# barlettacarmen/CrCNN

Hardware: AMD Instinct MI355X
Metric: encrypted images/sec (higher is better)
Workload: dtype u64

## Files before the change

crcnn_amd/csrc/kernels_mfma.hip:

```cpp
#include "kernels.h"
#include "limbred.h"
#include <cstdlib>

typedef int v4i __attribute__((ext_vector_type(4)));
typedef int v16i __attribute__((ext_vector_type(16)));
typedef signed char i8;

#define NPL 7
#define TILE_B (NPL * 64 * 32)

struct MfmaArgs {
    const i8 *xl; const i8 *wl; u64 *ys; const ModParams *mods; const u64 *bias;
    int xcdmap;
    int mfast;
    i8 *xl_out; int lp2; unsigned zdp_out;
    int n, k, B, zdp, npos, yd, xs, ys_, yf, yo, P, F, Fp, zblks, ksteps, M, mtiles, ntiles;
    unsigned img_bytes; unsigned long long wslot_bytes; int ksteps_real;
    int flat, S, zdc; unsigned fplane;
    int acc0[8][13];
    u64 qinv[8];
};

__device__ __forceinline__ void limb_digits(u64 r, u64 q, int (&d)[NPL])
{
    long long v = r > (q >> 1) ? (long long)r - (long long)q : (long long)r;
#pragma unroll
    for (int l = 0; l < NPL; l++) { d[l] = (int)(signed char)(v & 0xff); v = (v - d[l]) >> 8; }
}

template <int NST>
__global__ void __launch_bounds__(256) __attribute__((amdgpu_waves_per_eu(1, 1))) mfma_mac_kernel(MfmaArgs a)
{
    extern __shared__ __attribute__((aligned(16))) i8 lds[];
    const int lane = threadIdx.x & 63, wave = __builtin_amdgcn_readfirstlane(threadIdx.x >> 6), wm = wave >> 1, wn = wave & 1;
    const int slots = a.n * a.k, per = a.mtiles * a.ntiles;
    int g = blockIdx.x, slot, tile;
    if ((slots & 7) == 0) { const int xcd = g & 7, r = g >> 3; slot = xcd * (slots >> 3) + r / per; tile = r % per; }
    else { slot = g / per; tile = g % per; }
    const int mt = a.mfast ? tile % a.mtiles : tile / a.ntiles, nt = a.mfast ? tile / a.mtiles : tile % a.ntiles;
    const int i = slot / a.n, s = slot % a.n;
    const int m0 = mt * 64, f0 = nt * 64;
    const ModParams m = a.mods[i];
    const u64 qinv = a.qinv[i];
    const i8 *xs = a.xl + (size_t)slot * a.B * a.img_bytes;
    const i8 *ws = a.wl + (size_t)slot * a.wslot_bytes + (size_t)f0 * 32;
    u32 src_off[7];
#pragma unroll
    for (int j = 0; j < 7; j++) {
        const int pc = wave + 4 * j;
        if (pc < 14) {
            const int c16 = pc * 64 + lane;
            const int plane = c16 >> 7, row = (c16 >> 1) & 63, half = c16 & 1;
            const int mm = min(m0 + row, a.M - 1);
            const int b = mm / (2 * a.P), p = (mm >> 1) % a.P, c = mm & 1;
            const int ox = p / a.yo, oy = p % a.yo;
            src_off[j] = a.npos == 1 ? (u32)(plane * a.zblks * (2 * a.B) + mm) * 32 + half * 16
                       : a.flat ? (u32)b * a.img_bytes + (u32)(plane * a.fplane + (c * a.npos + (ox * a.xs) * a.yd + oy * a.ys_) * a.zdc + half * 16)
                                : (u32)b * a.img_bytes + (u32)(plane * (a.npos * 2 * a.zdp) + (((ox * a.xs) * a.yd + oy * a.ys_) * 2 + c) * a.zdp + half * 16);
        } else src_off[j] = (u32)(((pc - 14) >> 1) * (a.Fp * 32) + ((pc - 14) & 1) * 1024 + lane * 16);
    }
    const int kreal = a.ksteps_real;
    auto issue = [&](int ks) {
        const int ka = min(ks, kreal - 1);
        const int tap = ka / a.zblks, zb = ka - tap * a.zblks;
        const int kx = tap / a.yf, ky = tap - kx * a.yf;
        const int fkx = ka / a.S;
        const u32 delta = a.npos == 1 ? (u32)zb * (2 * a.B) * 32 : a.flat ? (u32)(fkx * a.yd * a.zdc + (ka - fkx * a.S) * 32) : (u32)((kx * a.yd + ky) * 2 * a.zdp + zb * 32);
        i8 *dst = lds + (ks % NST) * (2 * TILE_B);
        const i8 *wt = ws + (size_t)ks * (NPL * a.Fp * 32);
#pragma unroll
        for (int j = 0; j < 7; j++) {
            const int pc = wave + 4 * j;
            const i8 *src = pc < 14 ? xs + src_off[j] + delta : wt + src_off[j];
            __builtin_amdgcn_global_load_lds((const __attribute__((address_space(1))) void *)src, (__attribute__((address_space(3))) void *)(dst + pc * 1024), 16, 0, 0);
        }
    };
    v4i acc[2][2][13];
#pragma unroll
    for (int rs = 0; rs < 2; rs++)
#pragma unroll
        for (int cs = 0; cs < 2; cs++)
#pragma unroll
            for (int d = 0; d < 13; d++) { const int b0 = a.acc0[i][d]; acc[rs][cs][d] = v4i{b0, b0, b0, b0}; }
    const int K = a.ksteps;
#pragma unroll
    for (int j = 0; j < NST - 2; j++) if (j < K) issue(j);
    const int kg = lane >> 4, r16 = lane & 15;
    const int fragA = (wm * 32 + r16) * 32 + (kg & 1) * 16, fragW = (wn * 32 + r16) * 32 + (kg & 1) * 16;
    for (int ks = 0; ks < K; ks += 2) {
        const int younger = min(NST - 4, K - 2 - ks);
        if (younger >= 1) __builtin_amdgcn_s_waitcnt(7 | (7 << 4) | (15 << 8));
        else __builtin_amdgcn_s_waitcnt(0 | (7 << 4) | (15 << 8));
        __syncthreads();
        __builtin_amdgcn_sched_barrier(0);
        if (ks + NST - 2 < K) { issue(ks + NST - 2); __builtin_amdgcn_sched_barrier(0); if (ks + NST - 1 < K) issue(ks + NST - 1); }
        __builtin_amdgcn_sched_barrier(0);
        const i8 *tA = lds + ((ks + (kg >> 1)) % NST) * (2 * TILE_B), *tW = tA + TILE_B;
        v4i w[2][NPL], av[2 * NPL];
        auto read_a = [&](int gi) { return *reinterpret_cast<const v4i *>(tA + (gi % NPL) * (64 * 32) + fragA + (gi / NPL) * (16 * 32)); };
#pragma unroll
        for (int cs = 0; cs < 2; cs++)
#pragma unroll
            for (int l = 0; l < NPL; l++) w[cs][l] = *reinterpret_cast<const v4i *>(tW + l * (64 * 32) + fragW + cs * (16 * 32));
        av[0] = read_a(0); av[1] = read_a(1);
        __builtin_amdgcn_sched_barrier(0);
#pragma unroll
        for (int gi = 0; gi < 2 * NPL; gi++) {
            const int rs = gi / NPL, l = gi % NPL;
#pragma unroll
            for (int cs = 0; cs < 2; cs++)
#pragma unroll
                for (int mm = 0; mm < NPL; mm++)
                    acc[rs][cs][l + mm] = __builtin_amdgcn_mfma_i32_16x16x64_i8(av[gi], w[cs][mm], acc[rs][cs][l + mm], 0, 0, 0);
            if (gi + 2 < 2 * NPL) av[gi + 2] = read_a(gi + 2);
            __builtin_amdgcn_sched_barrier(0);
        }
    }
    u64 *yslot = a.ys + (size_t)slot * a.B * a.F * (2 * a.P);
    const u32 P2 = 2 * a.P;
    const u32 RL = 64 * a.P;
    if (a.xl_out) __syncthreads();
#pragma unroll
    for (int rs = 0; rs < 2; rs++) {
        const u32 mbase = m0 + wm * 32 + rs * 16 + 4 * kg, bb = mbase / P2, rem = mbase - bb * P2;
#pragma unroll
        for (int cs = 0; cs < 2; cs++) {
            const int fl = wn * 32 + cs * 16 + r16, f = f0 + fl;
            const u64 bv = (a.bias && f < a.F) ? a.bias[((size_t)f * a.k + i) * a.n + s] : 0;
#pragma unroll
            for (int reg = 0; reg < 4; reg++) {
                int D[13];
#pragma unroll
                for (int d = 0; d < 13; d++) D[d] = acc[rs][cs][d][reg];
                u64 v = diag_reduce_w(D, m, qinv);
                if ((reg & 1) == 0) v = addmod(v, bv, m.q);
                if (a.xl_out) {
                    const u32 rt = wm * 32 + rs * 16 + 4 * kg + reg, bl = rt >> a.lp2, qq = rt & (P2 - 1);
                    const u64 dg = f < a.F ? balanced_digit_bytes(v, m.q) : 0;
                    i8 *sp = lds + (size_t)bl * (NPL * 2 * RL) + (qq & 1) * RL + fl * a.P + (qq >> 1);
#pragma unroll
                    for (int l = 0; l < NPL; l++) sp[(size_t)l * (2 * RL)] = (i8)(dg >> (8 * l));
                } else {
                    const u32 r = rem + reg, b = bb + (r >= P2) + (r >= 2 * P2);
                    if (mbase + reg < (u32)a.M && f < a.F) yslot[b * (u32)(a.F - 1) * P2 + (u32)f * P2 + mbase + reg] = v;
                }
                __builtin_amdgcn_sched_barrier(0);
            }
        }
    }
    if (a.xl_out) {
        __syncthreads();
        const u32 imgs = 64 >> a.lp2, b0 = (u32)m0 >> a.lp2, per_run = RL / 16, pieces = imgs * NPL * 2 * per_run;
        const u32 ch0 = (u32)f0 * a.P;
        for (u32 o = threadIdx.x; o < pieces; o += 256) {
            const u32 run = o / per_run, off = (o - run * per_run) * 16, bl = run / (NPL * 2), lc = run - bl * (NPL * 2);
            const u32 ch = ch0 + off;
            if (b0 + bl < (u32)a.B && ch < a.zdp_out)
                *reinterpret_cast<uint4 *>(a.xl_out + (size_t)slot * ((size_t)NPL * 2 * a.B * a.zdp_out)
                                           + ((size_t)((lc >> 1) * (a.zdp_out / 32) + (ch >> 5)) * (2 * a.B) + (b0 + bl) * 2 + (lc & 1)) * 32 + (ch & 31)) =
                    *reinterpret_cast<const uint4 *>(lds + (size_t)run * RL + off);
        }
    }
}

#define TILE_A (NPL * 64 * 32)
template <int NST, int MODE>
__global__ void __launch_bounds__(256) __attribute__((amdgpu_waves_per_eu(2, 2))) mfma_mac2w_kernel(MfmaArgs a)
{
    extern __shared__ __attribute__((aligned(16))) i8 lds[];
    const int lane = threadIdx.x & 63, wave = __builtin_amdgcn_readfirstlane(threadIdx.x >> 6), wm = wave >> 1, wn = wave & 1;
    const int slots = a.n * a.k;
    const int fast = a.xcdmap ? (int)(blockIdx.x >> 3) : (int)blockIdx.x, slow = (int)blockIdx.y;
    const int slot = a.xcdmap ? (int)(blockIdx.x & 7) * (slots >> 3) + (int)blockIdx.z : (int)blockIdx.z;
    const int mt = a.mfast ? fast : slow, nt = a.mfast ? slow : fast;
    const int lgn = __builtin_ctz(a.n), i = slot >> lgn, s = slot & (a.n - 1);
    const int m0 = mt * 64, f0 = nt * 32;
    if (f0 >= a.F) return;
    const ModParams m = a.mods[i];
    const u64 qinv = a.qinv[i];
    const i8 *xs = a.xl + (size_t)slot * a.B * a.img_bytes;
    const int kg = lane >> 4, r16 = lane & 15;
    const i8 *wlane = a.wl + (size_t)slot * a.wslot_bytes + (size_t)(f0 + wn * 16 + r16) * 32 + (kg & 1) * 16 + (size_t)(kg >> 1) * (NPL * a.Fp * 32);
    const int wplane = a.Fp * 32, wstep = NPL * a.Fp * 32;
    u32 src_off[4]; int pcs[4];
    {
        const int row = ((wave & 1) << 5) + (lane >> 1), half = lane & 1;
        const int mm = min(m0 + row, a.M - 1);
        const int b = mm / (2 * a.P), rem = mm - b * (2 * a.P), p = rem >> 1, c = rem & 1;
        const int ox = p / a.yo, oy = p - ox * a.yo;
        const u32 rowpart = MODE == 0 ? (u32)mm * 32 + half * 16
                          : MODE == 1 ? (u32)b * a.img_bytes + (u32)((c * a.npos + (ox * a.xs) * a.yd + oy * a.ys_) * a.zdc + half * 16)
                                   : (u32)b * a.img_bytes + (u32)((((ox * a.xs) * a.yd + oy * a.ys_) * 2 + c) * a.zdp + half * 16);
        const u32 pstride = MODE == 0 ? (u32)(a.zblks * (2 * a.B)) * 32 : MODE == 1 ? a.fplane : (u32)(a.npos * 2 * a.zdp);
#pragma unroll
        for (int j = 0; j < 4; j++) {
            pcs[j] = wave + 4 * j < 14 ? wave + 4 * j : wave + 8;
            src_off[j] = rowpart + (u32)(pcs[j] >> 1) * pstride;
        }
    }
    const int kreal = a.ksteps_real;
    int iss = 0, ibuf = 0, zb = 0, ky = 0, kx = 0;
    u32 delta = 0;
    auto issue_a = [&](int ks) {
        (void)ks;
        i8 *dst = lds + ibuf * TILE_A;
#pragma unroll
        for (int j = 0; j < 4; j++)
            __builtin_amdgcn_global_load_lds((const __attribute__((address_space(1))) void *)(xs + src_off[j] + delta), (__attribute__((address_space(3))) void *)(dst + pcs[j] * 1024), 16, 0, 0);
        iss++; ibuf = ibuf + 1 == NST ? 0 : ibuf + 1;
        if (iss < kreal) {
            if (MODE == 0) delta += (u32)(2 * a.B) * 32;
            else if (MODE == 1) { if (++zb == a.S) { zb = 0; kx++; } delta = (u32)(kx * a.yd * a.zdc + zb * 32); }
            else { if (++zb == a.zblks) { zb = 0; if (++ky == a.yf) { ky = 0; kx++; } } delta = (u32)((kx * a.yd + ky) * 2 * a.zdp + zb * 32); }
        }
    };
    auto load_w = [&](int ks, v4i (&w)[NPL]) {
        const i8 *pw = wlane + (size_t)ks * wstep;
#pragma unroll
        for (int l = 0; l < NPL; l++) w[l] = *reinterpret_cast<const v4i *>(pw + (size_t)l * wplane);
    };
    v4i acc[2][13];
#pragma unroll
    for (int rs = 0; rs < 2; rs++)
#pragma unroll
        for (int d = 0; d < 13; d++) { const int b0 = a.acc0[i][d]; acc[rs][d] = v4i{b0, b0, b0, b0}; }
    const int K = a.ksteps;
    const int fragA = (wm * 32 + r16) * 32 + (kg & 1) * 16;
    auto dstep = [&](int ks, v4i (&wuse)[NPL], v4i (&wload)[NPL]) {
        if (ks + 2 < K) __builtin_amdgcn_s_waitcnt(11 | (7 << 4) | (15 << 8));
        else __builtin_amdgcn_s_waitcnt(0 | (7 << 4) | (15 << 8));
        __syncthreads();
        __builtin_amdgcn_sched_barrier(0);
        if (ks + 3 < K) issue_a(ks + 3);
        __builtin_amdgcn_sched_barrier(0);
        if (ks + 4 < K) { load_w(ks + 4, wload); __builtin_amdgcn_sched_barrier(0); issue_a(ks + 4); }
        __builtin_amdgcn_sched_barrier(0);
        const i8 *tA = lds + ((ks + (kg >> 1)) % NST) * TILE_A;
        v4i av[2 * NPL];
        auto read_a = [&](int gi) { return *reinterpret_cast<const v4i *>(tA + (gi % NPL) * (64 * 32) + fragA + (gi / NPL) * (16 * 32)); };
        av[0] = read_a(0); av[1] = read_a(1); av[2] = read_a(2);
        __builtin_amdgcn_sched_barrier(0);
#pragma unroll
        for (int gi = 0; gi < 2 * NPL; gi++) {
            const int rs = gi / NPL, l = gi % NPL;
#pragma unroll
            for (int mm = 0; mm < NPL; mm++)
                acc[rs][l + mm] = __builtin_amdgcn_mfma_i32_16x16x64_i8(av[gi], wuse[mm], acc[rs][l + mm], 0, 0, 0);
            if (gi + 3 < 2 * NPL) av[gi + 3] = read_a(gi + 3);
            __builtin_amdgcn_sched_barrier(0);
        }
    };
    v4i w0[NPL], w1[NPL], w2[NPL];
    issue_a(0); if (1 < K) issue_a(1);
    __builtin_amdgcn_sched_barrier(0);
    load_w(0, w0);
    __builtin_amdgcn_sched_barrier(0);
    if (2 < K) { issue_a(2); __builtin_amdgcn_sched_barrier(0); load_w(2, w1); }
    __builtin_amdgcn_sched_barrier(0);
    for (int ks = 0; ks < K; ks += 6) {
        dstep(ks, w0, w2);
        if (ks + 2 < K) dstep(ks + 2, w1, w0);
        if (ks + 4 < K) dstep(ks + 4, w2, w1);
    }
    u64 *yslot = a.ys + (size_t)slot * a.B * a.F * (2 * a.P);
    const u32 P2 = 2 * a.P;
    const u32 RL = 32 * a.P;
    if (a.xl_out) __syncthreads();
    const int fl = wn * 16 + r16, f = f0 + fl;
    const u64 bv = (a.bias && f < a.F) ? a.bias[((size_t)f * a.k + i) * a.n + s] : 0;
    const u32 img_jump = (u32)(a.F - 1) * P2;
#pragma unroll
    for (int rs = 0; rs < 2; rs++) {
        const u32 mbase = m0 + wm * 32 + rs * 16 + 4 * kg, bb = mbase / P2, rem = mbase - bb * P2;
        const u32 idx0 = bb * img_jump + (u32)f * P2 + mbase;
#pragma unroll
        for (int reg = 0; reg < 4; reg++) {
            int D[13];
#pragma unroll
            for (int d = 0; d < 13; d++) D[d] = acc[rs][d][reg];
            u64 v = diag_reduce_w(D, m, qinv);
            if ((reg & 1) == 0) v = addmod(v, bv, m.q);
            if (a.xl_out) {
                const u32 rt = wm * 32 + rs * 16 + 4 * kg + reg, bl = rt >> a.lp2, qq = rt & (P2 - 1);
                const u64 dg = f < a.F ? balanced_digit_bytes(v, m.q) : 0;
                i8 *sp = lds + (size_t)bl * (NPL * 2 * RL) + (qq & 1) * RL + fl * a.P + (qq >> 1);
#pragma unroll
                for (int l = 0; l < NPL; l++) sp[(size_t)l * (2 * RL)] = (i8)(dg >> (8 * l));
            } else {
                const u32 r = rem + reg, jump = (r >= P2 ? img_jump : 0u) + (r >= 2 * P2 ? img_jump : 0u);
                if (mbase + reg < (u32)a.M && f < a.F) yslot[idx0 + reg + jump] = v;
            }
            __builtin_amdgcn_sched_barrier(0);
        }
    }
    if (a.xl_out) {
        __syncthreads();
        const u32 imgs = 64 >> a.lp2, b0 = (u32)m0 >> a.lp2, per_run = RL / 16, pieces = imgs * NPL * 2 * per_run;
        const u32 ch0 = (u32)f0 * a.P;
        for (u32 o = threadIdx.x; o < pieces; o += 256) {
            const u32 run = o / per_run, off = (o - run * per_run) * 16, bl = run / (NPL * 2), lc = run - bl * (NPL * 2);
            const u32 ch = ch0 + off;
            if (b0 + bl < (u32)a.B && ch < a.zdp_out)
                *reinterpret_cast<uint4 *>(a.xl_out + (size_t)slot * ((size_t)NPL * 2 * a.B * a.zdp_out)
                                           + ((size_t)((lc >> 1) * (a.zdp_out / 32) + (ch >> 5)) * (2 * a.B) + (b0 + bl) * 2 + (lc & 1)) * 32 + (ch & 31)) =
                    *reinterpret_cast<const uint4 *>(lds + (size_t)run * RL + off);
        }
    }
}

__global__ void __launch_bounds__(64) limb_pack_tensor_kernel(const u64 *x, i8 *xl, const ModParams *mods, int n, int k, int B, int zd, int zdp, int npos, int packed, int group,
                                                              int Btot, int b0, int flat_zdc, unsigned flat_img)
{
    const int sblocks = n / 64;
    const int sb = blockIdx.x % (sblocks * k), i = sb / sblocks, s = (sb % sblocks) * 64 + threadIdx.x;
    const int zblks = zdp / 32;
    const size_t items = (size_t)B * npos * 2 * zblks;
    const u64 q = mods[i].q;
    for (size_t r0 = (size_t)(blockIdx.x / (sblocks * k)) * group, u = 0; u < (size_t)group && r0 + u < items; u++) {
        size_t r = r0 + u;
        int zb, c, pos, b;
        if (npos == 1) { const size_t rows = (size_t)B * 2; zb = (int)(r / rows); r %= rows; c = (int)(r & 1); b = (int)(r >> 1); pos = 0; }
        else { zb = (int)(r % zblks); r /= zblks; c = (int)(r % 2); r /= 2; pos = (int)(r % npos); b = (int)(r / npos); }
        u32 pl[NPL][8];
#pragma unroll
        for (int l = 0; l < NPL; l++)
#pragma unroll
            for (int wv = 0; wv < 8; wv++) pl[l][wv] = 0;
#pragma unroll
        for (int z = 0; z < 32; z++) {
            const int zz = zb * 32 + z;
            if (zz < zd) {
                u64 v = x[((((size_t)b * zd * npos + (size_t)zz * npos + pos) * 2 + c) * k + i) * (size_t)n + s];
                if (packed) v = (v & 0xffffffffULL) | ((v >> 32) << 28);
                int d[NPL]; limb_digits(v, q, d);
#pragma unroll
                for (int l = 0; l < NPL; l++) pl[l][z >> 2] |= (u32)(d[l] & 0xff) << (8 * (z & 3));
            }
        }
        if (flat_zdc) {
            i8 *dstf = xl + (((size_t)i * n + s) * Btot + b0 + b) * (size_t)flat_img + ((size_t)c * npos + pos) * flat_zdc;
#pragma unroll
            for (int l = 0; l < NPL; l++) {
                u32 *o = reinterpret_cast<u32 *>(dstf + (size_t)l * 2 * npos * flat_zdc);
#pragma unroll
                for (int wv = 0; wv < 8; wv++) if (wv * 4 < flat_zdc) o[wv] = pl[l][wv];
            }
            continue;
        }
        i8 *dst = npos == 1 ? xl + ((size_t)i * n + s) * ((size_t)NPL * 2 * Btot * zdp) + ((size_t)zb * (2 * Btot) + (b0 + b) * 2 + c) * 32
                            : xl + (((size_t)i * n + s) * Btot + b0 + b) * ((size_t)NPL * npos * 2 * zdp) + ((size_t)pos * 2 + c) * zdp + zb * 32;
        const size_t plane_stride = npos == 1 ? (size_t)zblks * (2 * Btot) * 32 : (size_t)npos * 2 * zdp;
#pragma unroll
        for (int l = 0; l < NPL; l++) {
            uint4 *o = reinterpret_cast<uint4 *>(dst + (size_t)l * plane_stride);
            o[0] = make_uint4(pl[l][0], pl[l][1], pl[l][2], pl[l][3]); o[1] = make_uint4(pl[l][4], pl[l][5], pl[l][6], pl[l][7]);
        }
    }
}
#define TRG 4
#define TSL 32
__global__ void __launch_bounds__(256) limb_pack_dense_kernel(const u64 *x, i8 *xl, const ModParams *mods, int n, int k, int B, int zd, int zdp, int packed, int Btot, int b0)
{
    __shared__ __attribute__((aligned(16))) i8 st[TSL * NPL * TRG * 32];
    const int sblocks = n / TSL, zblks = zdp / 32, rgs = (2 * B + TRG - 1) / TRG;
    const int sb = blockIdx.x % (sblocks * k), i = sb / sblocks, s0 = (sb % sblocks) * TSL;
    size_t r = blockIdx.x / (sblocks * k);
    const int rg = (int)(r % rgs), zb = (int)(r / rgs);
    const u64 q = mods[i].q;
    const int lane = threadIdx.x & (TSL - 1), qrow = (threadIdx.x >> 5) & (TRG - 1), h = threadIdx.x >> 7, row = rg * TRG + qrow;
    {
        u32 pl[NPL][4];
#pragma unroll
        for (int l = 0; l < NPL; l++)
#pragma unroll
            for (int wv = 0; wv < 4; wv++) pl[l][wv] = 0;
        if (row < 2 * B) {
            const int b = row >> 1, c = row & 1, z0 = zb * 32 + h * 16;
            const u64 *src = x + ((((size_t)b * zd + z0) * 2 + c) * k + i) * (size_t)n + s0 + lane;
#pragma unroll
            for (int z = 0; z < 16; z++)
                if (z0 + z < zd) {
                    u64 v = src[(size_t)z * 2 * k * n];
                    if (packed) v = (v & 0xffffffffULL) | ((v >> 32) << 28);
                    int d[NPL]; limb_digits(v, q, d);
#pragma unroll
                    for (int l = 0; l < NPL; l++) pl[l][z >> 2] |= (u32)(d[l] & 0xff) << (8 * (z & 3));
                }
        }
        i8 *sp = st + (size_t)lane * (NPL * TRG * 32) + qrow * 32 + h * 16;
#pragma unroll
        for (int l = 0; l < NPL; l++) *reinterpret_cast<uint4 *>(sp + l * (TRG * 32)) = make_uint4(pl[l][0], pl[l][1], pl[l][2], pl[l][3]);
    }
    __syncthreads();
    const int pieces_per_run = TRG * 2, rows_here = min(TRG, 2 * B - rg * TRG);
    const size_t plane_stride = (size_t)zblks * (2 * Btot) * 32, slot_stride = (size_t)NPL * plane_stride;
    for (int o = threadIdx.x; o < TSL * NPL * pieces_per_run; o += 256) {
        const int run = o / pieces_per_run, part = o - run * pieces_per_run, sl = run / NPL, l = run - sl * NPL;
        if ((part >> 1) >= rows_here) continue;
        i8 *dst = xl + ((size_t)i * n + s0 + sl) * slot_stride + (size_t)l * plane_stride + ((size_t)zb * (2 * Btot) + (size_t)b0 * 2 + rg * TRG) * 32 + part * 16;
        *reinterpret_cast<uint4 *>(dst) = *reinterpret_cast<const uint4 *>(st + (size_t)run * (TRG * 32) + part * 16);
    }
}
#define WFG 4
#define WSL 32
__global__ void __launch_bounds__(256) limb_pack_weights_kernel(const u64 *w, i8 *wl, const ModParams *mods, int n, int k, int F, int Fz, int Fp, int zd, int zblks, int xf, int yf, int f0,
                                                                int flat_zdc, int S)
{
    __shared__ __attribute__((aligned(16))) i8 st[WSL * NPL * WFG * 32];
    const int sblocks = n / WSL, taps = xf * yf, steps = flat_zdc ? xf * S : taps * zblks;
    const int sb = blockIdx.x % (sblocks * k), i = sb / sblocks, s0 = (sb % sblocks) * WSL;
    size_t r = blockIdx.x / (sblocks * k);
    const int step = (int)(r % steps); const int fg = (int)(r / steps);
    const ModParams m = mods[i];
    const u64 R = barrett128(0, 1, m);
    const int lane = threadIdx.x & (WSL - 1), fq = (threadIdx.x >> 5) & (WFG - 1), h = threadIdx.x >> 7, f = fg * WFG + fq;
    {
        u32 pl[NPL][4];
#pragma unroll
        for (int l = 0; l < NPL; l++)
#pragma unroll
            for (int wv = 0; wv < 4; wv++) pl[l][wv] = 0;
        if (f < F) {
            int tap, ch, ky = 0, kx = 0;
            if (flat_zdc) { kx = step / S; const int j0 = (step - kx * S) * 32 + h * 16; ky = j0 / flat_zdc; ch = j0 - ky * flat_zdc; tap = kx * yf + ky; }
            else { tap = step / zblks; ch = (step - tap * zblks) * 32 + h * 16; }
#pragma unroll
            for (int z = 0; z < 16; z++) {
                if (ch < zd && (!flat_zdc || ky < yf)) {
                    const u64 v = mulmod(w[((((size_t)f * zd + ch) * taps + tap) * k + i) * (size_t)n + s0 + lane], R, m);
                    int d[NPL]; limb_digits(v, m.q, d);
#pragma unroll
                    for (int l = 0; l < NPL; l++) pl[l][z >> 2] |= (u32)(d[l] & 0xff) << (8 * (z & 3));
                }
                ch++;
                if (flat_zdc && ch == flat_zdc) { ch = 0; ky++; tap++; }
            }
        }
        i8 *sp = st + (size_t)lane * (NPL * WFG * 32) + fq * 32 + h * 16;
#pragma unroll
        for (int l = 0; l < NPL; l++) *reinterpret_cast<uint4 *>(sp + l * (WFG * 32)) = make_uint4(pl[l][0], pl[l][1], pl[l][2], pl[l][3]);
    }
    __syncthreads();
    const int pieces_per_run = WFG * 2, filters_here = min(WFG, Fz - fg * WFG);
    const size_t slot_stride = (size_t)((steps + 1) & ~1) * NPL * Fp * 32;
    for (int o = threadIdx.x; o < WSL * NPL * pieces_per_run; o += 256) {
        const int run = o / pieces_per_run, part = o - run * pieces_per_run, sl = run / NPL, l = run - sl * NPL;
        if ((part >> 1) >= filters_here) continue;
        i8 *dst = wl + ((size_t)i * n + s0 + sl) * slot_stride + (size_t)step * (NPL * Fp * 32) + (size_t)l * Fp * 32 + (size_t)(f0 + fg * WFG) * 32 + part * 16;
// ... 12 lines not shown
        const int sl = r * 4 + ty;
        const size_t e = e0 + tx;
        tile[sl][tx] = e < rows ? ys[((size_t)i * n + s0 + sl) * rows + e] : 0;
    }
    __syncthreads();
#pragma unroll
    for (int r = 0; r < 16; r++) {
        const int el = r * 4 + ty;
        const size_t e = e0 + el;
        if (e < rows) { u64 v = tile[tx][el]; if (pack_out) v = (v & 0x0fffffffULL) | ((v >> 28) << 32); y[(e * k + i) * (size_t)n + s0 + tx] = v; }
    }
}
__global__ void __launch_bounds__(256) slotmajor_to_limb_kernel(const u64 *ys, i8 *xl, const ModParams *mods, int n, int B, int zd, int zdp, size_t total)
{
    const size_t t = (size_t)blockIdx.x * blockDim.x + threadIdx.x;
    if (t >= total) return;
    const int zgs = zdp / 16;
    const int zg = (int)(t % zgs); size_t r = t / zgs; const int c = (int)(r % 2); r /= 2; const int b = (int)(r % B); const size_t slot = r / B;
    const u64 q = mods[slot / n].q;
    u32 pl[NPL][4];
#pragma unroll
    for (int l = 0; l < NPL; l++)
#pragma unroll
        for (int wv = 0; wv < 4; wv++) pl[l][wv] = 0;
    const u64 *src = ys + (slot * B + b) * (size_t)zd * 2 + c;
#pragma unroll
    for (int z = 0; z < 16; z++) {
        const int zz = zg * 16 + z;
        if (zz < zd) {
            int d[NPL]; limb_digits(src[(size_t)zz * 2], q, d);
#pragma unroll
            for (int l = 0; l < NPL; l++) pl[l][z >> 2] |= (u32)(d[l] & 0xff) << (8 * (z & 3));
        }
    }
    i8 *dst = xl + slot * ((size_t)NPL * 2 * B * zdp) + ((size_t)(zg >> 1) * (2 * B) + b * 2 + c) * 32 + (zg & 1) * 16;
#pragma unroll
    for (int l = 0; l < NPL; l++) *reinterpret_cast<uint4 *>(dst + (size_t)l * (zdp / 32) * (2 * B) * 32) = make_uint4(pl[l][0], pl[l][1], pl[l][2], pl[l][3]);
}

static inline int round_up(int v, int m) { return (v + m - 1) / m * m; }
int k_limb_flat_zdc(int zd);
static void limb_tables(const crc_ctx *c, int T, int (*acc0)[13], u64 *qinv)
{
    for (int i = 0; i < c->k; i++) { limb_bias_table(c->tabs[i].m.q, T, acc0[i]); qinv[i] = inverse_mod_2_64(c->tabs[i].m.q); }
}

bool k_limb_supported(const crc_ctx *c, int T)
{
    if (c->n < 64 || T > 18000) return false;
    for (int i = 0; i < c->k; i++) if (c->tabs[i].m.bits > 55) return false;
    return true;
}
int k_limb_flat_zdc(int zd) { return zd < 32 ? round_up(zd, 4) : 0; }
int k_limb_steps(int zd, int xf, int yf) { const int zdc = k_limb_flat_zdc(zd); return zdc ? xf * ((yf * zdc + 31) / 32) : xf * yf * (round_up(zd, 32) / 32); }
static size_t limb_img_bytes(int zd, int npos) { const int zdc = k_limb_flat_zdc(zd); return zdc ? (size_t)round_up(NPL * 2 * npos * zdc, 16) : (size_t)NPL * npos * 2 * round_up(zd, 32); }
size_t k_limb_tensor_bytes(const crc_ctx *c, int B, int zd, int npos)
{
    if (npos == 1) return (size_t)c->n * c->k * B * NPL * 2 * round_up(zd, 32);
    return (size_t)c->n * c->k * B * limb_img_bytes(zd, npos) + 64;
}
size_t k_limb_weights_bytes(const crc_ctx *c, int nf, int zd, int xf, int yf) { return (size_t)c->n * c->k * round_up(k_limb_steps(zd, xf, yf), 2) * NPL * round_up(nf, 64) * 32; }
size_t k_limb_result_words(const crc_ctx *c, int B, int nf, int P) { return (size_t)c->n * c->k * B * nf * P * 2; }

int k_limb_pack_tensor(crc_ctx *c, const u64 *x, i8 *xl, int B, int zd, int npos, bool packed, hipStream_t st, int Btot, int b0)
{
    if (Btot <= 0) { Btot = B; b0 = 0; }
    if (b0 < 0 || b0 + B > Btot) return CRC_ERR_INVALID_ARGUMENT;
    const int zdp = round_up(zd, 32);
    const int group = c->tune.limb_pack_group > 1 ? c->tune.limb_pack_group : (npos == 1 && (B * 2) % 4 == 0 ? 4 : 1);
    const size_t items = (size_t)B * npos * 2 * (zdp / 32);
    if (npos == 1 && c->tune.limb_pack_group <= 1) {
        const size_t blocks = (size_t)(c->n / TSL) * c->k * (zdp / 32) * ((2 * (size_t)B + TRG - 1) / TRG);
        if (blocks == 0) return CRC_OK;
        if (blocks > 0x7fffffffULL) return CRC_ERR_INVALID_ARGUMENT;
        hipLaunchKernelGGL(limb_pack_dense_kernel, dim3((unsigned)blocks), dim3(256), 0, st, x, xl, c->d_mods, c->n, c->k, B, zd, zdp, packed ? 1 : 0, Btot, b0);
        HIPCHK(hipGetLastError());
        return CRC_OK;
    }
    const size_t blocks = (size_t)(c->n / 64) * c->k * ((items + group - 1) / group);
    if (blocks == 0) return CRC_OK;
    if (blocks > 0x7fffffffULL) return CRC_ERR_INVALID_ARGUMENT;
    const int fz = npos > 1 ? k_limb_flat_zdc(zd) : 0;
    hipLaunchKernelGGL(limb_pack_tensor_kernel, dim3((unsigned)blocks), dim3(64), 0, st, x, xl, c->d_mods, c->n, c->k, B, zd, zdp, npos, packed ? 1 : 0, group, Btot, b0, fz,
                       (unsigned)limb_img_bytes(zd, npos));
    HIPCHK(hipGetLastError());
    return CRC_OK;
}
int k_limb_pack_weights(crc_ctx *c, const u64 *w, i8 *wl, int nf, int zd, int xf, int yf, hipStream_t st, int f0, int ft)
{
    if (ft < 0) ft = nf;
    if (f0 < 0 || ft < 1 || f0 + ft > nf) return CRC_ERR_INVALID_ARGUMENT;
    const int zblks = round_up(zd, 32) / 32, Fp = round_up(nf, 64), zdc = k_limb_flat_zdc(zd), S = zdc ? (yf * zdc + 31) / 32 : 0;
    const size_t step = (size_t)NPL * Fp * 32, steps = (size_t)k_limb_steps(zd, xf, yf), slot = (size_t)round_up((int)steps, 2) * step;
    if (f0 == 0 && (steps & 1)) HIPCHK(hipMemset2DAsync(wl + steps * step, slot, 0, step, (size_t)c->n * c->k, st));
    const int fz = f0 + ft == nf ? Fp - f0 : ft;
    const size_t blocks = (size_t)(c->n / WSL) * c->k * ((fz + WFG - 1) / WFG) * steps;
    if (blocks > 0x7fffffffULL) return CRC_ERR_INVALID_ARGUMENT;
    hipLaunchKernelGGL(limb_pack_weights_kernel, dim3((unsigned)blocks), dim3(256), 0, st, w, wl, c->d_mods, c->n, c->k, ft, fz, Fp, zd, zblks, xf, yf, f0, zdc, S);
    HIPCHK(hipGetLastError());
    return CRC_OK;
}
int k_limb_result_to_rows(crc_ctx *c, const u64 *ys, u64 *y, size_t rows, bool pack_out, hipStream_t st)
{
    const size_t blocks = (size_t)(c->n / 64) * c->k * ((rows + 63) / 64);
    if (blocks == 0) return CRC_OK;
    if (blocks > 0x7fffffffULL) return CRC_ERR_INVALID_ARGUMENT;
    hipLaunchKernelGGL(slotmajor_to_rows_kernel, dim3((unsigned)blocks), dim3(256), 0, st, ys, y, c->n, c->k, rows, pack_out ? 1 : 0);
    HIPCHK(hipGetLastError());
    return CRC_OK;
}
int k_limb_result_to_limb(crc_ctx *c, const u64 *ys, i8 *xl, int B, int zd, hipStream_t st)
{
    const int zdp = round_up(zd, 32);
    const size_t total = (size_t)c->n * c->k * B * 2 * (zdp / 16);
    if (total == 0) return CRC_OK;
    hipLaunchKernelGGL(slotmajor_to_limb_kernel, dim3((unsigned)((total + 255) / 256)), dim3(256), 0, st, ys, xl, c->d_mods, c->n, B, zd, zdp, total);
    HIPCHK(hipGetLastError());
    return CRC_OK;
}
bool k_limb_direct_dense(int P) { const int p2 = 2 * P; return p2 <= 64 && (p2 & (p2 - 1)) == 0; }
int k_limb_mac(crc_ctx *c, const i8 *xl, const i8 *wl, u64 *ys, i8 *xl_out, const u64 *bias_ntt, int B, int zd, int xd, int yd, int xs, int ys_, int xf, int yf, int nf, hipStream_t st)
{
    if (B == 0) return CRC_OK;
    const int xo = (xd - xf) / xs + 1, yo = (yd - yf) / ys_ + 1;
    MfmaArgs a{};
    a.xl = xl; a.wl = wl; a.ys = ys; a.mods = c->d_mods; a.bias = bias_ntt;
    a.xl_out = nullptr; a.lp2 = -1; a.zdp_out = 0; a.mfast = 0;
    a.n = c->n; a.k = c->k; a.B = B; a.zdp = round_up(zd, 32); a.npos = xd * yd; a.yd = yd; a.xs = xs; a.ys_ = ys_; a.yf = yf; a.yo = yo; a.P = xo * yo;
    a.F = nf; a.Fp = round_up(nf, 64); a.zblks = a.zdp / 32; a.ksteps_real = k_limb_steps(zd, xf, yf); a.M = B * a.P * 2;
    a.mtiles = (a.M + 63) / 64; a.ntiles = a.Fp / 64;
    a.zdc = a.npos > 1 ? k_limb_flat_zdc(zd) : 0; a.flat = a.zdc ? 1 : 0; a.S = a.zdc ? (yf * a.zdc + 31) / 32 : 1; a.fplane = (unsigned)(2 * a.npos * a.zdc);
    const size_t img = a.npos == 1 ? (size_t)NPL * 2 * a.zdp : limb_img_bytes(zd, a.npos);
    if (img * B > 0xffffffffULL || !k_limb_supported(c, a.ksteps_real * 32)) return CRC_ERR_UNSUPPORTED;
    if (xl_out) {
        if (!k_limb_direct_dense(a.P)) return CRC_ERR_INVALID_ARGUMENT;
        a.xl_out = xl_out; a.zdp_out = (unsigned)round_up(nf * a.P, 32);
        for (a.lp2 = 0; (1 << a.lp2) < 2 * a.P; a.lp2++) {}
    }
    a.img_bytes = (unsigned)img; a.wslot_bytes = (unsigned long long)round_up(a.ksteps_real, 2) * NPL * a.Fp * 32;
    const size_t grid = (size_t)c->n * c->k * a.mtiles * a.ntiles;
    if (grid > 0x7fffffffULL) return CRC_ERR_INVALID_ARGUMENT;
    if (c->k > 8) return CRC_ERR_UNSUPPORTED;
    limb_tables(c, a.ksteps_real * 32, a.acc0, a.qinv);
    const int ring = c->tune.mfma_ring;
    a.ksteps = round_up(a.ksteps_real, 2);
    a.mfast = c->tune.mfma_order >= 0 ? c->tune.mfma_order : (a.mtiles < a.Fp / 32 ? 1 : 0);
    const int variant = c->tune.mfma_variant;
    if (variant == 2) {
        const int slots = c->n * c->k, ntiles2 = a.Fp / 32;
        a.xcdmap = (slots & 7) == 0 ? 1 : 0;
        const unsigned gfast = (unsigned)(a.mfast ? a.mtiles : ntiles2) * (a.xcdmap ? 8u : 1u), gslow = (unsigned)(a.mfast ? ntiles2 : a.mtiles), gz = (unsigned)(a.xcdmap ? slots >> 3 : slots);
        if (gslow > 65535u || gz > 65535u) return CRC_ERR_INVALID_ARGUMENT;
        const size_t lds = (size_t)5 * TILE_A;
        auto kern2 = a.npos == 1 ? mfma_mac2w_kernel<5, 0> : a.flat ? mfma_mac2w_kernel<5, 1> : mfma_mac2w_kernel<5, 2>;
        { const int rc = crc_ctx_ensure_lds(c, (const void *)kern2, lds); if (rc) return rc; }
        hipLaunchKernelGGL(kern2, dim3(gfast, gslow, gz), dim3(256), lds, st, a);
        HIPCHK(hipGetLastError());
        return CRC_OK;
    }
    const int nst = ring == 4 ? 4 : 5;
    const size_t lds = (size_t)nst * 2 * TILE_B;
    auto kern = nst == 4 ? mfma_mac_kernel<4> : mfma_mac_kernel<5>;
    { const int rc = crc_ctx_ensure_lds(c, (const void *)kern, lds); if (rc) return rc; }
    hipLaunchKernelGGL(kern, dim3((unsigned)grid), dim3(256), lds, st, a);
    HIPCHK(hipGetLastError());
    return CRC_OK;
}
```

crcnn_amd/csrc/limbred.h:

```cpp
#pragma once
#include "modarith.h"

CRC_HD u32 crc_alignbit(u32 hi, u32 lo, u32 sh)
{
#if defined(__HIP_DEVICE_COMPILE__)
    return __builtin_amdgcn_alignbit(hi, lo, sh);
#else
    return (u32)((((u64)hi << 32) | lo) >> sh);
#endif
}

CRC_HD u64 diag_reduce(const int (&D)[13], const ModParams &m, u64 qinv)
{
    typedef unsigned __int128 u128;
    const u128 s0 = ((u128)(((u64)(u32)D[12] << 32) | (u32)D[8]) << 64) | (((u64)(u32)D[4] << 32) | (u32)D[0]);
    const u128 s1 = ((u128)(u32)D[9] << 64) | (((u64)(u32)D[5] << 32) | (u32)D[1]);
    const u128 s2 = ((u128)(u32)D[10] << 64) | (((u64)(u32)D[6] << 32) | (u32)D[2]);
    const u128 s3 = ((u128)(u32)D[11] << 64) | (((u64)(u32)D[7] << 32) | (u32)D[3]);
    const u128 U = s0 + (s1 << 8) + (s2 << 16) + (s3 << 24);
    const u64 ulo = (u64)U, uhi = (u64)(U >> 64);
    const u64 mq = ulo * qinv;
    const u64 t = uhi - mulhi64(mq, m.q) + m.q;
    if (m.fold) {
        const u64 r = (t & (((u64)1 << m.bits) - 1)) + (u64)(u32)(t >> m.bits) * (u32)m.fold;
        return r >= m.q ? r - m.q : r;
    }
    return barrett128(t, 0, m);
}

CRC_HD u64 diag_reduce_w(const int (&D)[13], const ModParams &m, u64 qinv)
{
    typedef unsigned __int128 u128;
    const u32 a0 = (u32)D[1] << 8,  a1 = crc_alignbit((u32)D[5], (u32)D[1], 24), a2 = crc_alignbit((u32)D[9], (u32)D[5], 24),  a3 = (u32)D[9] >> 24;
    const u32 b0 = (u32)D[2] << 16, b1 = crc_alignbit((u32)D[6], (u32)D[2], 16), b2 = crc_alignbit((u32)D[10], (u32)D[6], 16), b3 = (u32)D[10] >> 16;
    const u32 c0 = (u32)D[3] << 24, c1 = crc_alignbit((u32)D[7], (u32)D[3], 8),  c2 = crc_alignbit((u32)D[11], (u32)D[7], 8),  c3 = (u32)D[11] >> 8;
    auto w128 = [](u32 w3, u32 w2, u32 w1, u32 w0) { return ((u128)(((u64)w3 << 32) | w2) << 64) | (((u64)w1 << 32) | w0); };
    const u128 U = w128((u32)D[12], (u32)D[8], (u32)D[4], (u32)D[0]) + w128(a3, a2, a1, a0) + w128(b3, b2, b1, b0) + w128(c3, c2, c1, c0);
    const u64 ulo = (u64)U, uhi = (u64)(U >> 64);
    const u64 mq = ulo * qinv;
    const u64 t = uhi - mulhi64(mq, m.q) + m.q;
    if (m.fold) {
        const u32 th = (u32)(t >> 32), sb = m.bits - 32;
        const u64 r = (((u64)(th & ((1u << sb) - 1)) << 32) | (u32)t) + (u64)(th >> sb) * (u32)m.fold;
        return r >= m.q ? r - m.q : r;
    }
    return barrett128(t, 0, m);
}

CRC_HD u64 diag_reduce_short(const int (&D)[13], u64 q, u64 qinv)
{
    u32 P[7];
    for (int j = 0; j < 6; j++) P[j] = (u32)D[2 * j] + ((u32)D[2 * j + 1] << 8);
    P[6] = (u32)D[12];
    const u32 o0 = P[1] << 16, o1 = (P[3] << 16) | (P[1] >> 16), o2 = (P[5] << 16) | (P[3] >> 16), o3 = P[5] >> 16;
    const u64 elo = ((u64)P[2] << 32) | P[0], ehi = ((u64)P[6] << 32) | P[4], olo = ((u64)o1 << 32) | o0, ohi = ((u64)o3 << 32) | o2;
    const u64 ulo = elo + olo, uhi = ehi + ohi + (ulo < elo);
    const u64 mq = ulo * qinv;
    const long long t = (long long)(uhi - mulhi64(mq, q));
    return (u64)(t + ((t >> 63) & (long long)q));
}

template <bool HAS_BIAS>
CRC_HD long long diag_reduce_short_centred(const int (&D)[13], u64 q, u64 qinv, long long bias_centred)
{
    typedef unsigned __int128 u128;
    u32 P[7];
    for (int j = 0; j < 6; j++) P[j] = (u32)D[2 * j] + ((u32)D[2 * j + 1] << 8);
    P[6] = (u32)D[12];
    const u128 E = ((u128)(((u64)P[6] << 32) | P[4]) << 64) | (((u64)P[2] << 32) | P[0]);
    const u128 O = ((u128)P[5] << 64) | (((u64)P[3] << 32) | P[1]);
    const u128 U = E + (O << 16);
    const u64 mq = (u64)U * qinv;
    long long t = (long long)((u64)(U >> 64) - mulhi64(mq, q));
    const long long h = (long long)(q >> 1);
    if (HAS_BIAS) t += bias_centred;
    t += t < -h ? (long long)q : 0;
    if (HAS_BIAS) t -= t > h ? (long long)q : 0;
    return t;
}
CRC_HD bool conv1_fold_ok(u64 q, u32 bits, u32 fold)
{
    typedef unsigned __int128 u128;
    if (bits < 53 || bits > 55 || fold == 0 || fold >= (1u << 26) || (((u64)1 << bits) - fold) != q) return false;
    const u128 uh_max = (((u128)0xC3) << 108) >> bits;
    return uh_max * fold + ((u128)1 << bits) < ((u128)1 << (bits + 32));
}
CRC_HD void diag_pack_words(const int (&D)[13], const u32 *PB, u32 (&u)[4])
{
    u32 P[7];
    for (int j = 0; j < 6; j++) P[j] = (u32)D[2 * j] + ((u32)D[2 * j + 1] << 8);
    P[6] = (u32)D[12];
    if (PB) for (int j = 0; j < 7; j++) P[j] += PB[j];
    const u32 o0 = P[1] << 16, o1 = crc_alignbit(P[3], P[1], 16), o2 = crc_alignbit(P[5], P[3], 16), o3 = P[5] >> 16;
    const u64 lo64 = (((u64)P[2] << 32) | P[0]) + (((u64)o1 << 32) | o0);
    const u64 hi64 = (((u64)P[6] << 32) | P[4]) + (((u64)o3 << 32) | o2) + (lo64 < (((u64)P[2] << 32) | P[0]));
    u[0] = (u32)lo64; u[1] = (u32)(lo64 >> 32); u[2] = (u32)hi64; u[3] = (u32)(hi64 >> 32);
}
CRC_HD long long fold_words_centred(u32 u0, u32 u1, u32 u2, u32 u3, u64 q, u32 bits, u32 fold, long long bias_centred)
{
    const u32 sb = bits - 32, m1 = (1u << sb) - 1;
    const u32 h0 = crc_alignbit(u2, u1, sb), h1 = crc_alignbit(u3, u2, sb);
    const u64 A = (u64)h0 * fold + (((u64)(u1 & m1) << 32) | u0);
    const u64 B = (u64)h1 * fold + (A >> 32);
    const u32 uh1 = crc_alignbit((u32)(B >> 32), (u32)B, sb);
    const u64 x2 = (u64)uh1 * fold + (((u64)((u32)B & m1) << 32) | (u32)A);
    u64 r = (u64)((u32)(x2 >> 32) >> sb) * fold + (((u64)((u32)(x2 >> 32) & m1) << 32) | (u32)x2);
    long long t = (long long)(r - q) + bias_centred;
    const long long h = (long long)(q >> 1);
    t += t < -h ? (long long)q : 0;
    t -= t > h ? (long long)q : 0;
    return t;
}
CRC_HD long long diag_fold_short_centred(const int (&D)[13], u64 q, u32 bits, u32 fold, long long bias_centred, const u32 *PB = nullptr)
{
    u32 u[4];
    diag_pack_words(D, PB, u);
    return fold_words_centred(u[0], u[1], u[2], u[3], q, bits, fold, bias_centred);
}
CRC_HD void diag7_pack_words(const int (&E)[7], const u32 *PB, u32 (&u)[3])
{
    u32 P[4];
    for (int j = 0; j < 3; j++) P[j] = (u32)E[2 * j] + ((u32)E[2 * j + 1] << 8);
    P[3] = (u32)E[6];
    if (PB) for (int j = 0; j < 4; j++) P[j] += PB[j];
    const u32 o0 = P[1] << 16, o1 = crc_alignbit(P[3], P[1], 16), o2 = P[3] >> 16;
    const u64 ev = ((u64)P[2] << 32) | P[0];
    const u64 lo64 = ev + (((u64)o1 << 32) | o0);
    u[0] = (u32)lo64; u[1] = (u32)(lo64 >> 32); u[2] = o2 + (lo64 < ev);
}
CRC_HD long long fold7_words_centred(u32 u0, u32 u1, u32 u2, u64 q, u32 bits, u32 fold, long long bias_centred)
{
    const u32 sb = bits - 32, m1 = (1u << sb) - 1;
    const u32 uh = crc_alignbit(u2, u1, sb);
    const u64 r = (u64)uh * fold + (((u64)(u1 & m1) << 32) | u0);
    long long t = (long long)(r - q) + bias_centred;
    const long long h = (long long)(q >> 1);
    t += t < -h ? (long long)q : 0;
    t -= t > h ? (long long)q : 0;
    return t;
}
CRC_HD long long diag7_fold_centred(const int (&E)[7], u64 q, u32 bits, u32 fold, long long bias_centred, const u32 *PB = nullptr)
{
    u32 u[3];
    diag7_pack_words(E, PB, u);
    return fold7_words_centred(u[0], u[1], u[2], q, bits, fold, bias_centred);
}
CRC_HD u64 centred_digit_bytes(long long cv) { return ((u64)cv + 0x0080808080808080ULL) ^ 0x0080808080808080ULL; }

CRC_HD u64 balanced_digit_bytes(u64 r, u64 q)
{
    const long long cv = r > (q >> 1) ? (long long)(r - q) : (long long)r;
    return ((u64)cv + 0x0080808080808080ULL) ^ 0x0080808080808080ULL;
}

inline u64 inverse_mod_2_64(u64 q) { u64 inv = q; for (int it = 0; it < 6; it++) inv *= 2 - q * inv; return inv; }

inline void bias_to_multiple(u64 q, long long (&B)[13])
{
    typedef unsigned __int128 u128;
    u128 K0 = 0;
    for (int d = 0; d < 13; d++) K0 += (u128)(u64)B[d] << (8 * d);
    const u64 rem = (u64)(K0 % q);
    long long delta = rem > q / 2 ? (long long)(q - rem) : -(long long)rem;
    for (int d = 0; d < 8 && delta; d++) { const long long dg = (long long)(signed char)(delta & 0xff); B[d] += dg; delta = (delta - dg) >> 8; }
}
inline void limb_bias_table(u64 q, int T, int (&out)[13])
{
    long long B[13];
    for (int d = 0; d < 13; d++) {
        const u64 bound = (u64)T * (u64)((d < 12 - d ? d : 12 - d) + 1) * 16384 + 256;
        u64 b = 1; while (b < bound) b <<= 1;
        B[d] = (long long)b;
    }
    bias_to_multiple(q, B);
    for (int d = 0; d < 13; d++) out[d] = (int)(u32)(u64)B[d];
}
inline void conv1_bias_table(u64 q, int (&out)[13])
{
    long long B[13];
    for (int d = 0; d < 13; d++) B[d] = d <= 10 ? 1 << 23 : d == 11 ? 1 << 21 : 1 << 19;
    bias_to_multiple(q, B);
    for (int d = 0; d < 13; d++) out[d] = (int)B[d];
}

inline void conv1_bias7_table(u64 q, int (&out)[7])
{
    typedef unsigned __int128 u128;
    long long B[7];
    u128 K0 = 0;
    for (int m = 0; m < 7; m++) { B[m] = 1 << 23; K0 += (u128)(u64)B[m] << (8 * m); }
    const u64 rem = (u64)(K0 % q);
    long long delta = rem > q / 2 ? (long long)(q - rem) : -(long long)rem;
    for (int m = 0; m < 7; m++) { const long long dg = (long long)(signed char)(delta & 0xff); B[m] += dg; delta = (delta - dg) >> 8; }
    for (int m = 0; m < 7; m++) out[m] = delta == 0 ? (int)B[m] : 0;
}
inline bool conv1_fold7_ok(u64 q, u32 bits, u32 fold)
{
    typedef unsigned __int128 u128;
    if (bits < 53 || bits > 55 || fold == 0 || fold >= (1u << 26) || (((u64)1 << bits) - fold) != q) return false;
// ... 10 lines not shown
```

Measured before the change: 793.4.

## Specialize MFMA epilogue for digit output with swapped operands and packed stores

```diff
diff --git a/crcnn_amd/csrc/kernels_mfma.hip b/crcnn_amd/csrc/kernels_mfma.hip
--- a/crcnn_amd/csrc/kernels_mfma.hip
+++ b/crcnn_amd/csrc/kernels_mfma.hip
@@ -163,10 +163,27 @@
     }
 }
 
+__device__ __forceinline__ void digit_words4(const long long (&cv)[4], const bool (&live)[4], u32 (&pl)[NPL])
+{
+    u32 lo[4], hi[4];
+#pragma unroll
+    for (int r = 0; r < 4; r++) { const u64 dg = live[r] ? centred_digit_bytes(cv[r]) : 0; lo[r] = (u32)dg; hi[r] = (u32)(dg >> 32); }
+    const u32 t0 = __builtin_amdgcn_perm(lo[1], lo[0], 0x05010400u), t1 = __builtin_amdgcn_perm(lo[1], lo[0], 0x07030602u);
+    const u32 u0 = __builtin_amdgcn_perm(lo[3], lo[2], 0x05010400u), u1 = __builtin_amdgcn_perm(lo[3], lo[2], 0x07030602u);
+    const u32 t2 = __builtin_amdgcn_perm(hi[1], hi[0], 0x05010400u), t3 = __builtin_amdgcn_perm(hi[1], hi[0], 0x07030602u);
+    const u32 u2 = __builtin_amdgcn_perm(hi[3], hi[2], 0x05010400u), u3 = __builtin_amdgcn_perm(hi[3], hi[2], 0x07030602u);
+    pl[0] = __builtin_amdgcn_perm(u0, t0, 0x05040100u); pl[1] = __builtin_amdgcn_perm(u0, t0, 0x07060302u);
+    pl[2] = __builtin_amdgcn_perm(u1, t1, 0x05040100u); pl[3] = __builtin_amdgcn_perm(u1, t1, 0x07060302u);
+    pl[4] = __builtin_amdgcn_perm(u2, t2, 0x05040100u); pl[5] = __builtin_amdgcn_perm(u2, t2, 0x07060302u);
+    pl[6] = __builtin_amdgcn_perm(u3, t3, 0x05040100u);
+}
+
 #define TILE_A (NPL * 64 * 32)
-template <int NST, int MODE>
+template <int NST, int MODE, int OUT>
 __global__ void __launch_bounds__(256) __attribute__((amdgpu_waves_per_eu(2, 2))) mfma_mac2w_kernel(MfmaArgs a)
 {
+    constexpr bool SWAP = OUT == 2 && MODE == 0;
+    constexpr bool PIXROWS = OUT == 2 && MODE != 0;
     extern __shared__ __attribute__((aligned(16))) i8 lds[];
     const int lane = threadIdx.x & 63, wave = __builtin_amdgcn_readfirstlane(threadIdx.x >> 6), wm = wave >> 1, wn = wave & 1;
     const int slots = a.n * a.k;
@@ -176,17 +193,24 @@
     const int lgn = __builtin_ctz(a.n), i = slot >> lgn, s = slot & (a.n - 1);
     const int m0 = mt * 64, f0 = nt * 32;
     if (f0 >= a.F) return;
-    const ModParams m = a.mods[i];
-    const u64 qinv = a.qinv[i];
     const i8 *xs = a.xl + (size_t)slot * a.B * a.img_bytes;
     const int kg = lane >> 4, r16 = lane & 15;
     const i8 *wlane = a.wl + (size_t)slot * a.wslot_bytes + (size_t)(f0 + wn * 16 + r16) * 32 + (kg & 1) * 16 + (size_t)(kg >> 1) * (NPL * a.Fp * 32);
     const int wplane = a.Fp * 32, wstep = NPL * a.Fp * 32;
+    auto load_w = [&](int ks, v4i (&w)[NPL]) {
+        const i8 *pw = wlane + (size_t)ks * wstep;
+#pragma unroll
+        for (int l = 0; l < NPL; l++) w[l] = *reinterpret_cast<const v4i *>(pw + (size_t)l * wplane);
+    };
+    v4i w0[NPL], w1[NPL], w2[NPL];
+    load_w(0, w0);
+    __builtin_amdgcn_sched_barrier(0);
     u32 src_off[4]; int pcs[4];
     {
         const int row = ((wave & 1) << 5) + (lane >> 1), half = lane & 1;
         const int mm = min(m0 + row, a.M - 1);
-        const int b = mm / (2 * a.P), rem = mm - b * (2 * a.P), p = rem >> 1, c = rem & 1;
+        const int b = PIXROWS ? mm >> a.lp2 : mm / (2 * a.P), rem = mm - b * (2 * a.P);
+        const int p = PIXROWS ? rem & (a.P - 1) : rem >> 1, c = PIXROWS ? rem >> (a.lp2 - 1) : rem & 1;
         const int ox = p / a.yo, oy = p - ox * a.yo;
         const u32 rowpart = MODE == 0 ? (u32)mm * 32 + half * 16
                           : MODE == 1 ? (u32)b * a.img_bytes + (u32)((c * a.npos + (ox * a.xs) * a.yd + oy * a.ys_) * a.zdc + half * 16)
@@ -214,16 +238,7 @@
             else { if (++zb == a.zblks) { zb = 0; if (++ky == a.yf) { ky = 0; kx++; } } delta = (u32)((kx * a.yd + ky) * 2 * a.zdp + zb * 32); }
         }
     };
-    auto load_w = [&](int ks, v4i (&w)[NPL]) {
-        const i8 *pw = wlane + (size_t)ks * wstep;
-#pragma unroll
-        for (int l = 0; l < NPL; l++) w[l] = *reinterpret_cast<const v4i *>(pw + (size_t)l * wplane);
-    };
     v4i acc[2][13];
-#pragma unroll
-    for (int rs = 0; rs < 2; rs++)
-#pragma unroll
-        for (int d = 0; d < 13; d++) { const int b0 = a.acc0[i][d]; acc[rs][d] = v4i{b0, b0, b0, b0}; }
     const int K = a.ksteps;
     const int fragA = (wm * 32 + r16) * 32 + (kg & 1) * 16;
     auto dstep = [&](int ks, v4i (&wuse)[NPL], v4i (&wload)[NPL]) {
@@ -245,55 +260,114 @@
             const int rs = gi / NPL, l = gi % NPL;
 #pragma unroll
             for (int mm = 0; mm < NPL; mm++)
-                acc[rs][l + mm] = __builtin_amdgcn_mfma_i32_16x16x64_i8(av[gi], wuse[mm], acc[rs][l + mm], 0, 0, 0);
+                acc[rs][l + mm] = SWAP ? __builtin_amdgcn_mfma_i32_16x16x64_i8(wuse[mm], av[gi], acc[rs][l + mm], 0, 0, 0)
+                                       : __builtin_amdgcn_mfma_i32_16x16x64_i8(av[gi], wuse[mm], acc[rs][l + mm], 0, 0, 0);
             if (gi + 3 < 2 * NPL) av[gi + 3] = read_a(gi + 3);
             __builtin_amdgcn_sched_barrier(0);
         }
     };
-    v4i w0[NPL], w1[NPL], w2[NPL];
     issue_a(0); if (1 < K) issue_a(1);
-    __builtin_amdgcn_sched_barrier(0);
-    load_w(0, w0);
     __builtin_amdgcn_sched_barrier(0);
     if (2 < K) { issue_a(2); __builtin_amdgcn_sched_barrier(0); load_w(2, w1); }
     __builtin_amdgcn_sched_barrier(0);
+    const ModParams m = a.mods[i];
+    const u64 qinv = a.qinv[i];
+#pragma unroll
+    for (int rs = 0; rs < 2; rs++)
+#pragma unroll
+        for (int d = 0; d < 13; d++) { const int b0 = a.acc0[i][d]; acc[rs][d] = v4i{b0, b0, b0, b0}; }
     for (int ks = 0; ks < K; ks += 6) {
         dstep(ks, w0, w2);
         if (ks + 2 < K) dstep(ks + 2, w1, w0);
         if (ks + 4 < K) dstep(ks + 4, w2, w1);
     }
-    u64 *yslot = a.ys + (size_t)slot * a.B * a.F * (2 * a.P);
     const u32 P2 = 2 * a.P;
     const u32 RL = 32 * a.P;
-    if (a.xl_out) __syncthreads();
-    const int fl = wn * 16 + r16, f = f0 + fl;
-    const u64 bv = (a.bias && f < a.F) ? a.bias[((size_t)f * a.k + i) * a.n + s] : 0;
-    const u32 img_jump = (u32)(a.F - 1) * P2;
-#pragma unroll
-    for (int rs = 0; rs < 2; rs++) {
-        const u32 mbase = m0 + wm * 32 + rs * 16 + 4 * kg, bb = mbase / P2, rem = mbase - bb * P2;
-        const u32 idx0 = bb * img_jump + (u32)f * P2 + mbase;
-#pragma unroll
-        for (int reg = 0; reg < 4; reg++) {
-            int D[13];
-#pragma unroll
-            for (int d = 0; d < 13; d++) D[d] = acc[rs][d][reg];
-            u64 v = diag_reduce_w(D, m, qinv);
-            if ((reg & 1) == 0) v = addmod(v, bv, m.q);
-            if (a.xl_out) {
-                const u32 rt = wm * 32 + rs * 16 + 4 * kg + reg, bl = rt >> a.lp2, qq = rt & (P2 - 1);
-                const u64 dg = f < a.F ? balanced_digit_bytes(v, m.q) : 0;
-                i8 *sp = lds + (size_t)bl * (NPL * 2 * RL) + (qq & 1) * RL + fl * a.P + (qq >> 1);
-#pragma unroll
-                for (int l = 0; l < NPL; l++) sp[(size_t)l * (2 * RL)] = (i8)(dg >> (8 * l));
-            } else {
+    const long long hq = (long long)(m.q >> 1);
+    if (OUT == 0) {
+        u64 *yslot = a.ys + (size_t)slot * a.B * a.F * P2;
+        const int f = f0 + wn * 16 + r16;
+        const u64 bv = (a.bias && f < a.F) ? a.bias[((size_t)f * a.k + i) * a.n + s] : 0;
+        const u32 img_jump = (u32)(a.F - 1) * P2;
+#pragma unroll
+        for (int rs = 0; rs < 2; rs++) {
+            const u32 mbase = m0 + wm * 32 + rs * 16 + 4 * kg, bb = mbase / P2, rem = mbase - bb * P2;
+            const u32 idx0 = bb * img_jump + (u32)f * P2 + mbase;
+#pragma unroll
+            for (int reg = 0; reg < 4; reg++) {
+                int D[13];
+#pragma unroll
+                for (int d = 0; d < 13; d++) D[d] = acc[rs][d][reg];
+                u64 v = diag_reduce_w(D, m, qinv);
+                if ((reg & 1) == 0) v = addmod(v, bv, m.q);
                 const u32 r = rem + reg, jump = (r >= P2 ? img_jump : 0u) + (r >= 2 * P2 ? img_jump : 0u);
                 if (mbase + reg < (u32)a.M && f < a.F) yslot[idx0 + reg + jump] = v;
+                __builtin_amdgcn_sched_barrier(0);
             }
-            __builtin_amdgcn_sched_barrier(0);
-        }
-    }
-    if (a.xl_out) {
+        }
+        return;
+    }
+    __syncthreads();
+    auto centred_bias = [&](int f, bool poly0) {
+        const u64 bv = (a.bias && poly0 && f < a.F) ? a.bias[((size_t)f * a.k + i) * a.n + s] : 0;
+        return bv > (u64)hq ? (long long)(bv - m.q) : (long long)bv;
+    };
+    if (SWAP) {
+        const int fl0 = wn * 16 + 4 * kg;
+        long long bc[4]; bool live[4];
+#pragma unroll
+        for (int reg = 0; reg < 4; reg++) { bc[reg] = centred_bias(f0 + fl0 + reg, (r16 & 1) == 0); live[reg] = f0 + fl0 + reg < a.F; }
+        i8 *sp = lds + (u32)(wm * 16 + (r16 >> 1)) * (NPL * 2 * 32) + (r16 & 1) * 32 + fl0;
+#pragma unroll
+        for (int rs = 0; rs < 2; rs++, sp += 8 * (NPL * 2 * 32)) {
+            long long cv[4];
+#pragma unroll
+            for (int reg = 0; reg < 4; reg++) {
+                int D[13];
+#pragma unroll
+                for (int d = 0; d < 13; d++) D[d] = acc[rs][d][reg];
+                cv[reg] = diag_reduce_w_centred(D, m, qinv, bc[reg]);
+                __builtin_amdgcn_sched_barrier(0);
+            }
+            u32 pl[NPL]; digit_words4(cv, live, pl);
+#pragma unroll
+            for (int l = 0; l < NPL; l++) *reinterpret_cast<u32 *>(sp + l * (2 * 32)) = pl[l];
+        }
+    } else {
+        const int fl = wn * 16 + r16, f = f0 + fl;
+        const long long bc = centred_bias(f, true);
+#pragma unroll
+        for (int rs = 0; rs < 2; rs++) {
+            const u32 rt0 = wm * 32 + rs * 16 + 4 * kg, bl = rt0 >> a.lp2, rem = rt0 & (P2 - 1);
+            long long cv[4];
+#pragma unroll
+            for (int reg = 0; reg < 4; reg++) {
+                int D[13];
+#pragma unroll
+                for (int d = 0; d < 13; d++) D[d] = acc[rs][d][reg];
+                const bool poly0 = PIXROWS ? rem < (u32)a.P : (reg & 1) == 0;
+                cv[reg] = diag_reduce_w_centred(D, m, qinv, poly0 ? bc : 0);
+                __builtin_amdgcn_sched_barrier(0);
+            }
+            if (PIXROWS) {
+                const bool lv = f < a.F, live[4] = {lv, lv, lv, lv};
+                u32 pl[NPL]; digit_words4(cv, live, pl);
+                i8 *sp = lds + bl * (NPL * 2 * RL) + (rem >> (a.lp2 - 1)) * RL + fl * a.P + (rem & (a.P - 1));
+#pragma unroll
+                for (int l = 0; l < NPL; l++) *reinterpret_cast<u32 *>(sp + l * (2 * RL)) = pl[l];
+            } else {
+#pragma unroll
+                for (int reg = 0; reg < 4; reg++) {
+                    const u32 r = rem + reg, qq = r & (P2 - 1);
+                    const u64 dg = f < a.F ? centred_digit_bytes(cv[reg]) : 0;
+                    i8 *sp = lds + (bl + (r >> a.lp2)) * (NPL * 2 * RL) + (qq & 1) * RL + fl * a.P + (qq >> 1);
+#pragma unroll
+                    for (int l = 0; l < NPL; l++) sp[l * (2 * RL)] = (i8)(dg >> (8 * l));
+                }
+            }
+        }
+    }
+    {
         __syncthreads();
         const u32 imgs = 64 >> a.lp2, b0 = (u32)m0 >> a.lp2, per_run = RL / 16, pieces = imgs * NPL * 2 * per_run;
         const u32 ch0 = (u32)f0 * a.P;
@@ -612,7 +686,10 @@
         const unsigned gfast = (unsigned)(a.mfast ? a.mtiles : ntiles2) * (a.xcdmap ? 8u : 1u), gslow = (unsigned)(a.mfast ? ntiles2 : a.mtiles), gz = (unsigned)(a.xcdmap ? slots >> 3 : slots);
         if (gslow > 65535u || gz > 65535u) return CRC_ERR_INVALID_ARGUMENT;
         const size_t lds = (size_t)5 * TILE_A;
-        auto kern2 = a.npos == 1 ? mfma_mac2w_kernel<5, 0> : a.flat ? mfma_mac2w_kernel<5, 1> : mfma_mac2w_kernel<5, 2>;
+        const int out = !a.xl_out ? 0 : (a.npos == 1 || a.P >= 4) ? 2 : 1;
+        auto kern2 = a.npos == 1 ? (out ? mfma_mac2w_kernel<5, 0, 2> : mfma_mac2w_kernel<5, 0, 0>)
+                   : a.flat ? (out == 2 ? mfma_mac2w_kernel<5, 1, 2> : out ? mfma_mac2w_kernel<5, 1, 1> : mfma_mac2w_kernel<5, 1, 0>)
+                            : (out == 2 ? mfma_mac2w_kernel<5, 2, 2> : out ? mfma_mac2w_kernel<5, 2, 1> : mfma_mac2w_kernel<5, 2, 0>);
         { const int rc = crc_ctx_ensure_lds(c, (const void *)kern2, lds); if (rc) return rc; }
         hipLaunchKernelGGL(kern2, dim3(gfast, gslow, gz), dim3(256), lds, st, a);
         HIPCHK(hipGetLastError());
diff --git a/crcnn_amd/csrc/limbred.h b/crcnn_amd/csrc/limbred.h
--- a/crcnn_amd/csrc/limbred.h
+++ b/crcnn_amd/csrc/limbred.h
@@ -28,7 +28,7 @@
     return barrett128(t, 0, m);
 }
 
-CRC_HD u64 diag_reduce_w(const int (&D)[13], const ModParams &m, u64 qinv)
+CRC_HD u64 diag_mont_w(const int (&D)[13], u64 q, u64 qinv)
 {
     typedef unsigned __int128 u128;
     const u32 a0 = (u32)D[1] << 8,  a1 = crc_alignbit((u32)D[5], (u32)D[1], 24), a2 = crc_alignbit((u32)D[9], (u32)D[5], 24),  a3 = (u32)D[9] >> 24;
@@ -38,13 +38,28 @@
     const u128 U = w128((u32)D[12], (u32)D[8], (u32)D[4], (u32)D[0]) + w128(a3, a2, a1, a0) + w128(b3, b2, b1, b0) + w128(c3, c2, c1, c0);
     const u64 ulo = (u64)U, uhi = (u64)(U >> 64);
     const u64 mq = ulo * qinv;
-    const u64 t = uhi - mulhi64(mq, m.q) + m.q;
-    if (m.fold) {
-        const u32 th = (u32)(t >> 32), sb = m.bits - 32;
-        const u64 r = (((u64)(th & ((1u << sb) - 1)) << 32) | (u32)t) + (u64)(th >> sb) * (u32)m.fold;
-        return r >= m.q ? r - m.q : r;
-    }
+    return uhi - mulhi64(mq, q) + q;
+}
+CRC_HD u64 fold_once_w(u64 t, u32 bits, u32 fold)
+{
+    const u32 th = (u32)(t >> 32), sb = bits - 32;
+    return (((u64)(th & ((1u << sb) - 1)) << 32) | (u32)t) + (u64)(th >> sb) * fold;
+}
+CRC_HD u64 diag_reduce_w(const int (&D)[13], const ModParams &m, u64 qinv)
+{
+    const u64 t = diag_mont_w(D, m.q, qinv);
+    if (m.fold) { const u64 r = fold_once_w(t, m.bits, m.fold); return r >= m.q ? r - m.q : r; }
     return barrett128(t, 0, m);
+}
+CRC_HD long long diag_reduce_w_centred(const int (&D)[13], const ModParams &m, u64 qinv, long long bias_centred)
+{
+    const u64 t = diag_mont_w(D, m.q, qinv);
+    const u64 r = m.fold ? fold_once_w(t, m.bits, m.fold) : barrett128(t, 0, m);
+    long long v = (long long)(r - m.q) + bias_centred;
+    const long long h = (long long)(m.q >> 1);
+    v += v < -h ? (long long)m.q : 0;
+    v -= v > h ? (long long)m.q : 0;
+    return v;
 }
 
 CRC_HD u64 diag_reduce_short(const int (&D)[13], u64 q, u64 qinv)
```

Result: slower. 772.5 (-2.6%).
